# mkangquantum/quits

Measured on AMD Instinct MI355X. Metric: decoded shots/sec + logical-error-rate, [[144,12,12]] BB code, d rounds, p=0.003, higher is better.
Workload: dtype f32

## Files before the change

quits_amd/csrc/bp_scatter_edge.h:

```cpp
#pragma once
#include "qd_internal.h"
#include <float.h>

__device__ __forceinline__ float qs_min_abs(float a, float b)
{
    float r;
    asm("v_min_f32 %0, %1, |%2|" : "=v"(r) : "v"(a), "v"(b));
    return r;
}
typedef uint32_t qs_u32x4 __attribute__((ext_vector_type(4)));
__device__ __forceinline__ uint4 qs_as_uint4(qs_u32x4 v) { return make_uint4(v.x, v.y, v.z, v.w); }
typedef __attribute__((address_space(3))) int32_t qs_lds_i32;
#define QS_LDS(off) ((qs_lds_i32 *)(uintptr_t)(uint32_t)(off))
#define QS_BIG 1.0e30f
#define QS_PRIO 1

#define QS_ACC(off) (*QS_LDS(off))
#define QS_SIGN_TOP (neww & 0x80000000u)
#define QS_HP1(A_) hp ^= (uint32_t)(A_);
#define QS_HPA(A_) hpa = (uint32_t)(A_);
#define QS_HPB(A_) hp = __builtin_amdgcn_bitop3_b32(hp, hpa, (uint32_t)(A_), 0x96);
#define QS_MAG_MASK(q_) (__builtin_amdgcn_inverse_ballot_w64(gsel_ & lq[q_]) ? s2 : s1)
#define QS_EDGE_M(off, k_, SGN_, TAILFIX, HP, MAG_)                                                          \
    {                                                                                                        \
        const int A_ = QS_ACC(off);                                                                          \
        const float mag_ = MAG_;                                                                             \
        const float prev_ = __uint_as_float((SGN_) | __float_as_uint(mag_));                                 \
        float d_ = (float)A_ - prev_;                                                                        \
        TAILFIX(d_, k_)                                                                                      \
        const float bm_ = d_ + 1.0f;                                                                         \
        HP(A_)                                                                                               \
        neww = __builtin_amdgcn_alignbit(neww, __float_as_uint(d_), 31);                                     \
                   \
        asm("v_cmp_lt_f32 vcc, |%1|, %2\n\tv_addc_co_u32 %0, vcc, %0, %0, vcc" : "+v"(ltw) : "v"(bm_), "v"(a1) : "vcc"); \
        a2 = __builtin_amdgcn_fmed3f(a1, a2, fabsf(bm_));                                                    \
        a1 = qs_min_abs(a1, bm_);                                                                            \
    }
__device__ __forceinline__ float qs_min_f32(float a, float b)
{
    float r;
    asm("v_min_f32 %0, %1, %2" : "=v"(r) : "v"(a), "v"(b));
    return r;
}
#define QS_KEY_POS0 0x3F800000u
#define QS_KEY_LIMIT 262144.0f
#define QS_EDGE_K(off, k_, SGN_, TAILFIX, HP, MAG_)                                                          \
    {                                                                                                        \
        const int A_ = QS_ACC(off);                                                                          \
        const float mag_ = MAG_;                                                                             \
        const float prev_ = __uint_as_float((SGN_) | __float_as_uint(mag_));                                 \
        float d_ = (float)A_ - prev_;                                                                        \
        TAILFIX(d_, k_)                                                                                      \
        const float bm_ = d_ + 1.0f;                                                                         \
        HP(A_)                                                                                               \
        neww = __builtin_amdgcn_alignbit(neww, __float_as_uint(d_), 31);                                     \
        const float key_ = fabsf(bm_) + __uint_as_float(QS_KEY_POS0 + ((uint32_t)(k_) << 17));               \
        a2 = __builtin_amdgcn_fmed3f(a1, a2, key_);                                                          \
        a1 = qs_min_f32(a1, key_);                                                                           \
    }
#define QS_KEYS_DECODE(trip_)                                                                                \
    const bool keys_ok_ = __builtin_amdgcn_ballot_w64(!(a2 < QS_KEY_LIMIT)) == 0ull;                         \
    {                                                                                                        \
        const float f1_ = __builtin_floorf(a1), f2_ = __builtin_floorf(a2);                                  \
        kst = min((uint32_t)((a1 - f1_) * 64.0f), (uint32_t)max((trip_) - 1, 0));                            \
        a1 = f1_ - 1.0f; a2 = f2_ - 1.0f;                                                                    \
    }
#define QS_CMP_EDGE QS_EDGE_M
#define QS_CMP_PAD { neww <<= 1; ltw <<= 1; }
#define QS_CMP_WORD_BEGIN uint32_t ltw = 0u;
#define QS_CMP_WORD_END(k0_, kend_) if (ltw) kst = (uint32_t)((k0_) + (kend_) - 1 - (int)__builtin_ctz(ltw));
#define QS_CMP_END(trip_)
#define QS_KEY_EDGE QS_EDGE_K
#define QS_KEY_PAD { neww <<= 1; }
#define QS_KEY_WORD_BEGIN
#define QS_KEY_WORD_END(k0_, kend_)
#define QS_KEY_END(trip_) QS_KEYS_DECODE(trip_)
#define QS_NOFIX(x_, k_)
#define QS_TAILFIX(x_, k_) x_ = ((int)(k_) < dc) ? x_ : QS_BIG;

#define QS_ADD(off, v_) (void)__hip_atomic_fetch_add(QS_LDS(off), v_, __ATOMIC_RELAXED, __HIP_MEMORY_SCOPE_WORKGROUP);
#define QS_SCAT(off, k_, bit_, TAILFIX)                                                                      \
    {                                                                                                        \
        const int sm_ = __builtin_amdgcn_sbfe((int)own, bit_, 1);                                            \
        int v_ = (int)__builtin_amdgcn_bitop3_b32((uint32_t)n1, (uint32_t)nx, (uint32_t)sm_, 0x78);           \
        TAILFIX(v_, k_)                                                                                      \
        QS_ADD(off, v_)                                                                                      \
    }
#define QS_TAILZERO(v_, k_) v_ = ((int)(k_) < dc) ? v_ : 0;

template <int NW>
__device__ __forceinline__ void qs_reset_to_priors(const int32_t *prior_g, uint32_t offA, int nslots, int tid)
{
    const int nbytes = nslots * 4;
    const int lane16 = (tid & 63) * 16;
    for (int p = __builtin_amdgcn_readfirstlane(tid >> 6) * 1024; p < nbytes; p += NW * 1024)
        if (p + lane16 < nbytes)
            __builtin_amdgcn_global_load_lds((const __attribute__((address_space(1))) void *)(reinterpret_cast<const char *>(prior_g) + p + lane16),
                                             (__attribute__((address_space(3))) void *)(uintptr_t)(offA + (uint32_t)p), 16, 0, 0);
}
```

quits_amd/csrc/bp_scatter_wide.hip:

```cpp
#include "qd_internal.h"
#include "qd_host.h"
#include "../../include/quits_amd.h"
#include "bp_scatter_edge.h"

#define QSW_GATHER_PRIO(j_) if ((j_) == 0) __builtin_amdgcn_s_setprio(0); else if ((j_) == CPL - 1) __builtin_amdgcn_s_setprio(2); else __builtin_amdgcn_s_setprio(1);

template <int T, int MW, int CPL, int NSW>
__global__ void __launch_bounds__(T, MW) qd_bp_scatter_wide_kernel(BpGraphDev g, ScatGraphDev sg, DecodeArgs a, ScatArgs x)
{
    extern __shared__ __align__(16) unsigned char smem[];
    const uint32_t lds_base = (uint32_t)(uintptr_t)(__attribute__((address_space(3))) unsigned char *)smem;
    if (lds_base != 0u) __builtin_trap();
    uint32_t *outw = reinterpret_cast<uint32_t *>(smem + sg.off_out);
    int *misc = reinterpret_cast<int *>(smem + sg.off_misc);
    constexpr int NW = T / 64;
    static_assert(T % 64 == 0 && NW <= 16, "workgroup shape");

    const int tid = threadIdx.x;
    const int64_t shot = blockIdx.x;
    const uint8_t *det = a.det + shot * a.det_stride + a.det_offset;
    const uint8_t *upd = a.upd ? a.upd + shot * a.upd_stride : nullptr;
    const int m_pad = g.m_pad, n_pad = g.n_pad;

    int any = 0;
    uint32_t synd[CPL];
    int dcs[CPL];
    bool act[CPL];
    if (tid < 64) misc[tid] = 0;
    int cs[CPL];
#pragma unroll
    for (int j = 0; j < CPL; ++j) {
        const int sw = __builtin_amdgcn_readfirstlane(sg.wave_map[j * NW + (tid >> 6)]);
        const int c = sw * 64 + (tid & 63);
        cs[j] = c;
        act[j] = sw >= 0 && c < g.m;
        synd[j] = 0u; dcs[j] = 0;
        if (act[j]) {
            const uint32_t o = g.chk_orig[c];
            synd[j] = det[o] & 1u;
            if (upd && (int)o < a.upd_rows) synd[j] ^= upd[o] & 1u;
            any |= (int)synd[j];
            dcs[j] = sg.chk_deg[c];
        }
    }
    int dws[CPL];
#pragma unroll
    for (int j = 0; j < CPL; ++j) {
        const int wslot = __builtin_amdgcn_readfirstlane(cs[j] >> 6);
        dws[j] = wslot >= 0 ? (int)sg.deg_w[wslot] : 0;
    }
    qs_reset_to_priors<NW>(x.prior_g, (uint32_t)sg.offA, sg.nslots, tid);
    for (int w = tid; w < g.out_words; w += T) outw[w] = 0u;
    __syncthreads();
    any = qd_block_or(any, misc, NW, 0);
    if (!any) {
        for (int w = tid; w < g.out_words; w += T) a.err_bits[shot * g.out_words + w] = 0u;
        if (tid == 0) a.status[shot] = QD_STATUS_CONVERGED | QD_STATUS_ZERO | a.status_or;
        return;
    }
    float S1[CPL], S2[CPL], A1[CPL], A2[CPL], mx2 = 0.f;
    uint32_t KOLD[CPL], KST[CPL], O[CPL][NSW], Q[CPL][NSW];
    [[maybe_unused]] uint32_t cmpf = 0u;
#pragma unroll
    for (int j = 0; j < CPL; ++j) {
        S1[j] = 0.f; S2[j] = 0.f; A1[j] = FLT_MAX; A2[j] = FLT_MAX; KOLD[j] = 0xFFFFFFFFu; KST[j] = 0u;
#pragma unroll
        for (int w = 0; w < NSW; ++w) { O[j][w] = 0u; Q[j][w] = 0u; }
    }
    const uint32_t cur = (uint32_t)sg.offA;
    const __amdgpu_buffer_rsrc_t adj_rsrc = __builtin_amdgcn_make_buffer_rsrc((void *)sg.adjA, 0, (g.max_rdeg_pad / 4 + 2) * m_pad * 16, 0x00020000);
    const int adj_row = m_pad * 16;
#define QS_ADJ(row_) qs_as_uint4(__builtin_amdgcn_raw_buffer_load_b128(adj_rsrc, adj_voff, (row_) * adj_row, 0))
#define QS_ADJ_FIRST qs_as_uint4(__builtin_amdgcn_raw_buffer_load_b128(adj_rsrc, cs[0] * 16, 0, 0))
    uint4 pf = QS_ADJ_FIRST;
    const bool fast = x.first_pass != nullptr && a.max_iter >= 1;
    bool have = false;
    if (fast) {
#pragma unroll
        for (int j = 0; j < CPL; ++j)
            if (act[j]) {
                const uint4 *rp = reinterpret_cast<const uint4 *>(x.first_pass) + 2 * cs[j];
                const uint4 r0 = rp[0], r1 = rp[1];
                const uint32_t negw[3] = {r0.w, r1.x, r1.y};
                const uint32_t flip = 0u - ((synd[j] ^ r1.z) & 1u);
                A1[j] = __uint_as_float(r0.x); A2[j] = __uint_as_float(r0.y); KST[j] = r0.z;
#pragma unroll
                for (int w = 0; w < NSW; ++w) Q[j][w] = negw[w] ^ flip;
                mx2 = fmaxf(mx2, A2[j]);
            }
        have = true;
    }
#define QSW_VOTE(us_, anyun_)                                                                          \
        {                                                                                              \
            const unsigned long long bal = __ballot(us_);                                              \
            if ((tid & 63) == 0) misc[32 + (tid >> 6)] = (bal != 0ull);                                \
        }                                                                                              \
        __syncthreads();                                                                               \
        anyun_ = 0;                                                                                    \
        {                                                                                              \
            const int4 *f4 = reinterpret_cast<const int4 *>(misc + 32);                                \
            for (int w = 0; w < (NW + 3) / 4; ++w) {                                                   \
                const int4 v = f4[w];                                                                  \
                anyun_ |= v.x | v.y | v.z | v.w;                                                       \
            }                                                                                          \
        }
    int t = 0, converged = 0;
    for (;;) {
      if (!have) {
        bool us = false;
        if (fast && t == a.max_iter) break;
#pragma unroll
        for (int j = 0; j < CPL; ++j) {
            float a1 = FLT_MAX, a2 = FLT_MAX;
            uint32_t kst = 0u;
            QSW_GATHER_PRIO(j)
#define QSW_WALKED                                                                                     \
                {                                                                                      \
                    const uint32_t flip = 0u - ((synd[j] ^ (uint32_t)__popc(par)) & 1u);               \
                    _Pragma("unroll")                                                                  \
                    for (int w = 0; w < NSW; ++w) Q[j][w] = neg[w] ^ flip;                             \
                    mx2 = fmaxf(mx2, a2);                                                              \
                    us = us || (((synd[j] ^ (hp >> 31)) & 1u) != 0u);                                  \
                }
            bool cmpw = true;
            if constexpr (NSW == 2) cmpw = __builtin_amdgcn_ballot_w64((cmpf >> j) & 1u) != 0ull;
#ifdef QSW_STATS
            if ((tid & 63) == 0 && __ballot(act[j])) atomicAdd(&a.dbg[14], 1ull);
#endif
            if (act[j]) {
                if constexpr (NSW == 2) {
                    if (!cmpw) {
#define QS_WALK(p_) QS_KEY_##p_
#include "bp_scatter_wide_walk.inc"
#undef QS_WALK
                        if (keys_ok_) QSW_WALKED
                        else { cmpw = true; cmpf |= 1u << j; a1 = FLT_MAX; a2 = FLT_MAX; kst = 0u; }
                    }
                }
                if (cmpw) {
#ifdef QSW_STATS
                    if ((tid & 63) == 0) atomicAdd(&a.dbg[15], 1ull);
#endif
#define QS_WALK(p_) QS_CMP_##p_
#include "bp_scatter_wide_walk.inc"
#undef QS_WALK
                    QSW_WALKED
                }
            }
#undef QSW_WALKED
            A1[j] = a1; A2[j] = a2; KST[j] = kst;
        }
        __builtin_amdgcn_s_setprio(0);
        pf = QS_ADJ_FIRST;
        int anyun;
        QSW_VOTE(us, anyun)
        if (t >= 1 && !anyun) { converged = 1; break; }
        if (t == a.max_iter) break;
        qs_reset_to_priors<NW>(x.prior_g, cur, sg.nslots, tid);
        __syncthreads();
      }
        have = false;
        __builtin_amdgcn_s_setprio(QS_PRIO);
#pragma unroll
        for (int j = 0; j < CPL; ++j) {
#ifdef QSW_STATS
            {
                bool same = A1[j] == S1[j] && A2[j] == S2[j] && (KST[j] == KOLD[j] || A1[j] == A2[j]);
#pragma unroll
                for (int w = 0; w < NSW; ++w) same = same && Q[j][w] == O[j][w];
                const unsigned long long ba = __ballot(act[j]), bs = __ballot(act[j] && same);
                if ((tid & 63) == 0 && ba) {
                    const int bk = min(t / 10, 4);
                    atomicAdd(&a.dbg[0], 1ull); atomicAdd(&a.dbg[2 + bk], 1ull);
                    if (bs == ba) { atomicAdd(&a.dbg[1], 1ull); atomicAdd(&a.dbg[7 + bk], 1ull); }
                    atomicAdd(&a.dbg[12], (unsigned long long)__popcll(bs)); atomicAdd(&a.dbg[13], (unsigned long long)__popcll(ba));
                }
            }
#endif
            if (act[j]) {
                int dwj = dws[j];
                asm volatile("" : "+s"(dwj));
                const int trip = dwj & 0xFF, wmax = (dwj >> 8) & 0xFF, wmin = (dwj >> 16) & 0xFF, wmin4 = wmin & ~3;
                const int adj_voff = cs[j] * 16;
                const int dc = dcs[j];
                const int n1 = (int)A1[j], nx = n1 ^ -n1;
                const uint32_t kst = KST[j];
                const uint32_t fixn_off = __builtin_amdgcn_raw_buffer_load_b32(adj_rsrc, (int)((kst >> 2) * (uint32_t)adj_row + (kst & 3u) * 4u) + adj_voff, 0, 0);
                const int ng = trip >> 2;
#define QS_GROUP_POS(gi_) const int b0_ = kendw - 1 - 4 * ((gi_) - 8 * w);
#define QS_GROUP_PLAIN(e4, gi_)                                                                                                      \
                {                                                                                                                    \
                    QS_GROUP_POS(gi_)                                                                                                \
                    QS_SCAT(e4.x, 0, b0_, QS_NOFIX) QS_SCAT(e4.y, 0, b0_ - 1, QS_NOFIX) QS_SCAT(e4.z, 0, b0_ - 2, QS_NOFIX) QS_SCAT(e4.w, 0, b0_ - 3, QS_NOFIX) \
                }
#define QS_SCAT_TAIL(off, q_)                                                                                                        \
                    if (k + (q_) < wmin) QS_SCAT(off, 0, b0_ - (q_), QS_NOFIX)                                                       \
                    else if (k + (q_) < wmax) QS_SCAT(off, k + (q_), b0_ - (q_), QS_TAILZERO)
#define QS_GROUP_TAIL(e4, gi_)                                                                                                       \
                {                                                                                                                    \
                    const int k = (gi_) * 4;                                                                                         \
                    QS_GROUP_POS(gi_)                                                                                                \
                    QS_SCAT_TAIL(e4.x, 0) QS_SCAT_TAIL(e4.y, 1) QS_SCAT_TAIL(e4.z, 2) QS_SCAT_TAIL(e4.w, 3)                          \
                }
#pragma unroll
                for (int w = 0; w < NSW; ++w) {
                    if (32 * w < trip) {
                        const int kendw = min(trip - 32 * w, 32);
                        const uint32_t own = Q[j][w];
                        const int g1 = min(ng, 8 * w + 8);
                        const int gp = min(g1, max(wmin4 >> 2, 8 * w));
                        uint4 ea = (j == 0 && w == 0) ? pf : QS_ADJ(8 * w), eb;
                        int gi = 8 * w;
#pragma unroll 1
                        for (; gi + 2 <= gp; gi += 2) {
                            eb = QS_ADJ(gi + 1);
                            QS_GROUP_PLAIN(ea, gi)
                            ea = QS_ADJ(gi + 2);
                            QS_GROUP_PLAIN(eb, gi + 1)
                        }
#pragma unroll 1
                        for (; gi < gp; ++gi) {
                            const uint4 e4 = ea;
                            ea = QS_ADJ(gi + 1);
                            QS_GROUP_PLAIN(e4, gi)
                        }
#pragma unroll 1
                        for (; gi + 1 < g1; ++gi) {
                            const uint4 e4 = ea;
                            ea = QS_ADJ(gi + 1);
                            QS_GROUP_TAIL(e4, gi)
                        }
                        if (gi < g1) QS_GROUP_TAIL(ea, gi)
                    }
                }
#undef QS_GROUP_PLAIN
#undef QS_GROUP_TAIL
#undef QS_SCAT_TAIL
#undef QS_GROUP_POS
                {
                    const int kw = (int)(kst >> 5), kendw = min(trip - 32 * kw, 32);
                    uint32_t wd = Q[j][0];
#pragma unroll
                    for (int w = 1; w < NSW; ++w) wd = (kw == w) ? Q[j][w] : wd;
                    const uint32_t sg_ = (wd >> (kendw - 1 - (int)(kst & 31u))) & 1u;
                    const int dlt = (int)A2[j] - n1;
                    const int vn = sg_ ? -dlt : dlt;
                    (void)__hip_atomic_fetch_add(QS_LDS(fixn_off), vn, __ATOMIC_RELAXED, __HIP_MEMORY_SCOPE_WORKGROUP);
                }
            }
            S1[j] = A1[j]; S2[j] = A2[j]; KOLD[j] = KST[j];
#pragma unroll
            for (int w = 0; w < NSW; ++w) O[j][w] = Q[j][w];
        }
        __builtin_amdgcn_s_setprio(0);
        pf = QS_ADJ_FIRST;
        __syncthreads();
        ++t;
    }
    if (fast && !converged) {
        bool us = false;
#pragma unroll
        for (int j = 0; j < CPL; ++j) {
            QSW_GATHER_PRIO(j)
            if (act[j]) {
                int dwj = dws[j];
                asm volatile("" : "+s"(dwj));
                const int ng = (dwj & 0xFF) >> 2;
                const int adj_voff = cs[j] * 16;
                uint32_t hp = 0u, hpa = 0u;
#define QS_HP_GROUP(e4) { QS_HPA(QS_ACC(e4.x)) QS_HPB(QS_ACC(e4.y)) QS_HPA(QS_ACC(e4.z)) QS_HPB(QS_ACC(e4.w)) }
                uint4 nx = (j == 0) ? pf : QS_ADJ(0);
                int gi = 0;
#pragma unroll 1
                for (; gi + 2 <= ng; gi += 2) {
                    const uint4 eb = QS_ADJ(gi + 1);
                    QS_HP_GROUP(nx)
                    nx = QS_ADJ(gi + 2);
                    QS_HP_GROUP(eb)
                }
                if (gi < ng) QS_HP_GROUP(nx)
#undef QS_HP_GROUP
                us = us || (((synd[j] ^ (hp >> 31)) & 1u) != 0u);
            }
        }
        __builtin_amdgcn_s_setprio(0);
        int anyun;
        QSW_VOTE(us, anyun)
        if (!anyun) converged = 1;
    }
#undef QSW_VOTE
#undef QS_ADJ
#undef QS_ADJ_FIRST
#undef QSW_GATHER_PRIO

    {
        const int tripped = qd_block_or(!(mx2 < x.m2_limit) ? 1 : 0, misc, NW, 0);
        if (tripped) {
            if (tid == 0) {
                const int at = atomicAdd(x.recheck_count, 1);
                if (at < x.recheck_cap) x.recheck_list[at] = (int32_t)shot;
            }
            return;
        }
    }
    for (int b = tid; b < sg.nslots; b += T)
        if (*QS_LDS(cur + 4u * (uint32_t)b) < 0) {
            const uint32_t jf = sg.slot_fault[b];
            if (jf != 0xFFFFFFFFu) atomicOr(&outw[jf >> 5], 1u << (jf & 31u));
        }
    if (!converged && a.want_llr && tid == 0) misc[48] = atomicAdd(a.fail_count, 1);
    __syncthreads();
    for (int w = tid; w < g.out_words; w += T) a.err_bits[shot * g.out_words + w] = outw[w];
    if (!converged && a.want_llr) {
        const int slot = misc[48];
        float *dst = a.llr_ws + (int64_t)slot * n_pad;
        for (int k1 = tid; k1 < g.n; k1 += T) dst[k1] = (float)(*QS_LDS(cur + 4u * sg.k1_slot[k1]) + 1) * x.grid_inv;
        if (tid == 0) a.fail_list[slot] = (int32_t)shot;
    }
    if (tid == 0) a.status[shot] = t | (converged * QD_STATUS_CONVERGED) | a.status_or;
}

#undef QS_ACC
#define QS_ACC(off) (prior_g[((uint32_t)(off) - (uint32_t)sg.offA) >> 2])
#define QS_ADJ(row_) qs_as_uint4(__builtin_amdgcn_raw_buffer_load_b128(adj_rsrc, adj_voff, (row_) * adj_row, 0))
template <int NSW>
__global__ void __launch_bounds__(64) qd_bp_first_pass_kernel(BpGraphDev g, ScatGraphDev sg, const int32_t *prior_g, uint32_t *rec)
{
    static_assert(NSW == 3, "the record has room for three sign words");
    const int c = (int)blockIdx.x * 64 + (int)threadIdx.x;
    const bool actv = c < g.m;
    constexpr int j = 0;
    const int cs[1] = {c}, dws[1] = {__builtin_amdgcn_readfirstlane((int)sg.deg_w[blockIdx.x])}, dcs[1] = {actv ? (int)sg.chk_deg[c] : 0};
    const float S1[1] = {0.f}, S2[1] = {0.f};
    const uint32_t KOLD[1] = {0xFFFFFFFFu}, O[1][NSW] = {{0u, 0u, 0u}};
    const __amdgpu_buffer_rsrc_t adj_rsrc = __builtin_amdgcn_make_buffer_rsrc((void *)sg.adjA, 0, (g.max_rdeg_pad / 4 + 2) * g.m_pad * 16, 0x00020000);
    const int adj_row = g.m_pad * 16;
    const uint4 pf = qs_as_uint4(__builtin_amdgcn_raw_buffer_load_b128(adj_rsrc, c * 16, 0, 0));
    float a1 = FLT_MAX, a2 = FLT_MAX;
    uint32_t kst = 0u;
    uint4 r0 = make_uint4(__float_as_uint(FLT_MAX), __float_as_uint(FLT_MAX), 0u, 0u);
    uint4 r1 = make_uint4(0u, 0u, 0u, (uint32_t)sg.offA + (uint32_t)(sg.nslots - 32 + (int)(threadIdx.x & 31)) * 4u);
    if (actv) {
#define QS_WALK(p_) QS_CMP_##p_
#include "bp_scatter_wide_walk.inc"
#undef QS_WALK
        (void)hp;
        r0 = make_uint4(__float_as_uint(a1), __float_as_uint(a2), kst, neg[0]);
        r1 = make_uint4(neg[1], neg[2], (uint32_t)__popc(par) & 1u,
                        __builtin_amdgcn_raw_buffer_load_b32(adj_rsrc, (int)((kst >> 2) * (uint32_t)adj_row + (kst & 3u) * 4u) + c * 16, 0, 0));
    }
    uint4 *out = reinterpret_cast<uint4 *>(rec) + 2 * c;
    out[0] = r0; out[1] = r1;
}
#undef QS_ADJ
#undef QS_ACC

hipError_t qd_launch_bp_first_pass(const BpGraphDev &g, const ScatGraphDev &sg, const int32_t *prior_g, uint32_t *rec, hipStream_t s)
{
    if (g.max_rdeg_pad > 96 || g.m_pad % 64) return hipErrorInvalidValue;
    hipLaunchKernelGGL(qd_bp_first_pass_kernel<3>, dim3((unsigned)(g.m_pad / 64)), dim3(64), 0, s, g, sg, prior_g, rec);
    return hipGetLastError();
}

template <int T, int MW, int CPL, int NSW>
static hipError_t launch_scatter_wide_t(const BpGraphDev &g, const ScatGraphDev &sg, const DecodeArgs &a, const ScatArgs &x, int64_t B, hipStream_t s)
{
    auto k = qd_bp_scatter_wide_kernel<T, MW, CPL, NSW>;
    hipError_t e = hipFuncSetAttribute((const void *)k, hipFuncAttributeMaxDynamicSharedMemorySize, sg.lds_bytes);
    if (e != hipSuccess) return e;
    hipLaunchKernelGGL(k, dim3((unsigned)B), dim3(T), sg.lds_bytes, s, g, sg, a, x);
    return hipGetLastError();
}

hipError_t qd_launch_bp_scatter_wide(const BpGraphDev &g, const ScatGraphDev &sg, const DecodeArgs &a, const ScatArgs &x, int64_t B, hipStream_t s)
{
    const bool two_words = g.max_rdeg_pad <= 64;
    switch (sg.wide_threads * 8 + sg.wide_cpl) {
    case 512 * 8 + 2:
        return two_words ? launch_scatter_wide_t<512, 8, 2, 2>(g, sg, a, x, B, s) : hipErrorInvalidValue;
    case 256 * 8 + 2:
        return two_words ? launch_scatter_wide_t<256, 8, 2, 2>(g, sg, a, x, B, s) : hipErrorInvalidValue;
    case 128 * 8 + 2:
        return two_words ? launch_scatter_wide_t<128, 8, 2, 2>(g, sg, a, x, B, s) : hipErrorInvalidValue;
    case 256 * 8 + 1:
        return two_words ? launch_scatter_wide_t<256, 8, 1, 2>(g, sg, a, x, B, s) : hipErrorInvalidValue;
    case 512 * 8 + 1:
        return two_words ? launch_scatter_wide_t<512, 8, 1, 2>(g, sg, a, x, B, s) : hipErrorInvalidValue;
    case 1024 * 8 + 1:
        return two_words ? launch_scatter_wide_t<1024, 8, 1, 2>(g, sg, a, x, B, s) : hipErrorInvalidValue;
    case 704 * 8 + 2:
        return launch_scatter_wide_t<704, 6, 2, 3>(g, sg, a, x, B, s);
    case 1024 * 8 + 2: return launch_scatter_wide_t<1024, 4, 2, 3>(g, sg, a, x, B, s);
    case 512 * 8 + 3: return launch_scatter_wide_t<512, 4, 3, 3>(g, sg, a, x, B, s);
    default: return hipErrorInvalidValue;
    }
}
```

Baseline: 1.824 million.

## Merge per-check state arrays, prefetch fix address, and streamline convergence vote

Drops the separate A1/A2/KST/Q state arrays and writes gather results directly into S1/S2/KOLD/O, which removes the end-of-iteration copy and reduces register pressure. The fix-node LDS address load is issued early, after the gather phase and before the barrier, instead of inside the scatter phase. The syndrome is stored in the sign bit so the unsatisfied-check vote becomes a single bitop3 and a sign-bit ballot, and the cross-wave vote read is reduced to one int2/int4 load. The signed fix-up uses an sbfe mask instead of a branch. The risk is subtle correctness changes in the reworked bit-position and sign logic.

Measured after the change: 1.855 million, median of 6. 1.7% higher.

```diff
diff --git a/quits_amd/csrc/bp_scatter_edge.h b/quits_amd/csrc/bp_scatter_edge.h
--- a/quits_amd/csrc/bp_scatter_edge.h
+++ b/quits_amd/csrc/bp_scatter_edge.h
@@ -40,6 +40,12 @@
 {
     float r;
     asm("v_min_f32 %0, %1, %2" : "=v"(r) : "v"(a), "v"(b));
+    return r;
+}
+__device__ __forceinline__ float qs_max_f32(float a, float b)
+{
+    float r;
+    asm("v_max_f32 %0, %1, %2" : "=v"(r) : "v"(a), "v"(b));
     return r;
 }
 #define QS_KEY_POS0 0x3F800000u
diff --git a/quits_amd/csrc/bp_scatter_wide.hip b/quits_amd/csrc/bp_scatter_wide.hip
--- a/quits_amd/csrc/bp_scatter_wide.hip
+++ b/quits_amd/csrc/bp_scatter_wide.hip
@@ -39,6 +39,7 @@
             const uint32_t o = g.chk_orig[c];
             synd[j] = det[o] & 1u;
             if (upd && (int)o < a.upd_rows) synd[j] ^= upd[o] & 1u;
+            synd[j] <<= 31;
             any |= (int)synd[j];
             dcs[j] = sg.chk_deg[c];
         }
@@ -58,20 +59,31 @@
         if (tid == 0) a.status[shot] = QD_STATUS_CONVERGED | QD_STATUS_ZERO | a.status_or;
         return;
     }
-    float S1[CPL], S2[CPL], A1[CPL], A2[CPL], mx2 = 0.f;
-    uint32_t KOLD[CPL], KST[CPL], O[CPL][NSW], Q[CPL][NSW];
+    float S1[CPL], S2[CPL], mx2 = 0.f;
+    uint32_t KOLD[CPL], O[CPL][NSW];
+    uint32_t FX[CPL];
+#ifdef QSW_STATS
+    float P1[CPL], P2[CPL];
+    uint32_t PK[CPL], PO[CPL][NSW];
+#endif
     [[maybe_unused]] uint32_t cmpf = 0u;
 #pragma unroll
     for (int j = 0; j < CPL; ++j) {
-        S1[j] = 0.f; S2[j] = 0.f; A1[j] = FLT_MAX; A2[j] = FLT_MAX; KOLD[j] = 0xFFFFFFFFu; KST[j] = 0u;
-#pragma unroll
-        for (int w = 0; w < NSW; ++w) { O[j][w] = 0u; Q[j][w] = 0u; }
+        S1[j] = 0.f; S2[j] = 0.f; KOLD[j] = 0xFFFFFFFFu; FX[j] = 0u;
+#pragma unroll
+        for (int w = 0; w < NSW; ++w) O[j][w] = 0u;
+#ifdef QSW_STATS
+        P1[j] = 0.f; P2[j] = 0.f; PK[j] = 0xFFFFFFFFu;
+#pragma unroll
+        for (int w = 0; w < NSW; ++w) PO[j][w] = 0u;
+#endif
     }
     const uint32_t cur = (uint32_t)sg.offA;
     const __amdgpu_buffer_rsrc_t adj_rsrc = __builtin_amdgcn_make_buffer_rsrc((void *)sg.adjA, 0, (g.max_rdeg_pad / 4 + 2) * m_pad * 16, 0x00020000);
     const int adj_row = m_pad * 16;
 #define QS_ADJ(row_) qs_as_uint4(__builtin_amdgcn_raw_buffer_load_b128(adj_rsrc, adj_voff, (row_) * adj_row, 0))
 #define QS_ADJ_FIRST qs_as_uint4(__builtin_amdgcn_raw_buffer_load_b128(adj_rsrc, cs[0] * 16, 0, 0))
+#define QS_FIX_ADDR(j_) __builtin_amdgcn_raw_buffer_load_b32(adj_rsrc, (int)(__umul24(KOLD[j_] >> 2, (uint32_t)adj_row) + (KOLD[j_] & 3u) * 4u) + cs[j_] * 16, 0, 0)
     uint4 pf = QS_ADJ_FIRST;
     const bool fast = x.first_pass != nullptr && a.max_iter >= 1;
     bool have = false;
@@ -82,32 +94,32 @@
                 const uint4 *rp = reinterpret_cast<const uint4 *>(x.first_pass) + 2 * cs[j];
                 const uint4 r0 = rp[0], r1 = rp[1];
                 const uint32_t negw[3] = {r0.w, r1.x, r1.y};
-                const uint32_t flip = 0u - ((synd[j] ^ r1.z) & 1u);
-                A1[j] = __uint_as_float(r0.x); A2[j] = __uint_as_float(r0.y); KST[j] = r0.z;
-#pragma unroll
-                for (int w = 0; w < NSW; ++w) Q[j][w] = negw[w] ^ flip;
-                mx2 = fmaxf(mx2, A2[j]);
+                const uint32_t flip = 0u - (((synd[j] >> 31) ^ r1.z) & 1u);
+                S1[j] = __uint_as_float(r0.x); S2[j] = __uint_as_float(r0.y); KOLD[j] = r0.z; FX[j] = r1.w;
+#pragma unroll
+                for (int w = 0; w < NSW; ++w) O[j][w] = negw[w] ^ flip;
+                mx2 = qs_max_f32(mx2, S2[j]);
             }
         have = true;
     }
-#define QSW_VOTE(us_, anyun_)                                                                          \
+#define QSW_VOTE_ROUND(uw_, synd_, hp_) uw_ = __builtin_amdgcn_bitop3_b32(uw_, synd_, hp_, 0xF6);
+#define QSW_VOTE(uw_, anyun_)                                                                          \
         {                                                                                              \
-            const unsigned long long bal = __ballot(us_);                                              \
-            if ((tid & 63) == 0) misc[32 + (tid >> 6)] = (bal != 0ull);                                \
+            const unsigned long long bal = __ballot((int)(uw_) < 0);                                   \
+            if ((tid & 63) == 0) reinterpret_cast<unsigned char *>(misc + 32)[tid >> 6] = (unsigned char)(bal != 0ull); \
         }                                                                                              \
         __syncthreads();                                                                               \
-        anyun_ = 0;                                                                                    \
-        {                                                                                              \
-            const int4 *f4 = reinterpret_cast<const int4 *>(misc + 32);                                \
-            for (int w = 0; w < (NW + 3) / 4; ++w) {                                                   \
-                const int4 v = f4[w];                                                                  \
-                anyun_ |= v.x | v.y | v.z | v.w;                                                       \
-            }                                                                                          \
+        if constexpr (NW <= 8) {                                                                       \
+            const int2 v = *reinterpret_cast<const int2 *>(misc + 32);                                 \
+            anyun_ = v.x | v.y;                                                                        \
+        } else {                                                                                       \
+            const int4 v = *reinterpret_cast<const int4 *>(misc + 32);                                 \
+            anyun_ = (v.x | v.y) | (v.z | v.w);                                                        \
         }
     int t = 0, converged = 0;
     for (;;) {
       if (!have) {
-        bool us = false;
+        uint32_t us = 0u;
         if (fast && t == a.max_iter) break;
 #pragma unroll
         for (int j = 0; j < CPL; ++j) {
@@ -116,16 +128,19 @@
             QSW_GATHER_PRIO(j)
 #define QSW_WALKED                                                                                     \
                 {                                                                                      \
-                    const uint32_t flip = 0u - ((synd[j] ^ (uint32_t)__popc(par)) & 1u);               \
+                    const uint32_t flip = 0u - ((uint32_t)__popc(par ^ synd[j]) & 1u);                 \
                     _Pragma("unroll")                                                                  \
-                    for (int w = 0; w < NSW; ++w) Q[j][w] = neg[w] ^ flip;                             \
-                    mx2 = fmaxf(mx2, a2);                                                              \
-                    us = us || (((synd[j] ^ (hp >> 31)) & 1u) != 0u);                                  \
+                    for (int w = 0; w < NSW; ++w) O[j][w] = neg[w] ^ flip;                             \
+                    mx2 = qs_max_f32(mx2, a2);                                                         \
+                    QSW_VOTE_ROUND(us, synd[j], hp)                                                    \
                 }
             bool cmpw = true;
             if constexpr (NSW == 2) cmpw = __builtin_amdgcn_ballot_w64((cmpf >> j) & 1u) != 0ull;
 #ifdef QSW_STATS
             if ((tid & 63) == 0 && __ballot(act[j])) atomicAdd(&a.dbg[14], 1ull);
+            P1[j] = S1[j]; P2[j] = S2[j]; PK[j] = KOLD[j];
+#pragma unroll
+            for (int w = 0; w < NSW; ++w) PO[j][w] = O[j][w];
 #endif
             if (act[j]) {
                 if constexpr (NSW == 2) {
@@ -148,10 +163,13 @@
                 }
             }
 #undef QSW_WALKED
-            A1[j] = a1; A2[j] = a2; KST[j] = kst;
+            S1[j] = a1; S2[j] = a2; KOLD[j] = kst;
         }
         __builtin_amdgcn_s_setprio(0);
         pf = QS_ADJ_FIRST;
+#pragma unroll
+        for (int j = 0; j < CPL; ++j)
+            if (act[j]) FX[j] = QS_FIX_ADDR(j);
         int anyun;
         QSW_VOTE(us, anyun)
         if (t >= 1 && !anyun) { converged = 1; break; }
@@ -165,9 +183,9 @@
         for (int j = 0; j < CPL; ++j) {
 #ifdef QSW_STATS
             {
-                bool same = A1[j] == S1[j] && A2[j] == S2[j] && (KST[j] == KOLD[j] || A1[j] == A2[j]);
-#pragma unroll
-                for (int w = 0; w < NSW; ++w) same = same && Q[j][w] == O[j][w];
+                bool same = S1[j] == P1[j] && S2[j] == P2[j] && (KOLD[j] == PK[j] || S1[j] == S2[j]);
+#pragma unroll
+                for (int w = 0; w < NSW; ++w) same = same && O[j][w] == PO[j][w];
                 const unsigned long long ba = __ballot(act[j]), bs = __ballot(act[j] && same);
                 if ((tid & 63) == 0 && ba) {
                     const int bk = min(t / 10, 4);
@@ -183,9 +201,9 @@
                 const int trip = dwj & 0xFF, wmax = (dwj >> 8) & 0xFF, wmin = (dwj >> 16) & 0xFF, wmin4 = wmin & ~3;
                 const int adj_voff = cs[j] * 16;
                 const int dc = dcs[j];
-                const int n1 = (int)A1[j], nx = n1 ^ -n1;
-                const uint32_t kst = KST[j];
-                const uint32_t fixn_off = __builtin_amdgcn_raw_buffer_load_b32(adj_rsrc, (int)((kst >> 2) * (uint32_t)adj_row + (kst & 3u) * 4u) + adj_voff, 0, 0);
+                const int n1 = (int)S1[j], nx = n1 ^ -n1;
+                const uint32_t kst = KOLD[j];
+                const uint32_t fixn_off = FX[j];
                 const int ng = trip >> 2;
 #define QS_GROUP_POS(gi_) const int b0_ = kendw - 1 - 4 * ((gi_) - 8 * w);
 #define QS_GROUP_PLAIN(e4, gi_)                                                                                                      \
@@ -206,7 +224,7 @@
                 for (int w = 0; w < NSW; ++w) {
                     if (32 * w < trip) {
                         const int kendw = min(trip - 32 * w, 32);
-                        const uint32_t own = Q[j][w];
+                        const uint32_t own = O[j][w];
                         const int g1 = min(ng, 8 * w + 8);
                         const int gp = min(g1, max(wmin4 >> 2, 8 * w));
                         uint4 ea = (j == 0 && w == 0) ? pf : QS_ADJ(8 * w), eb;
@@ -238,19 +256,20 @@
 #undef QS_SCAT_TAIL
 #undef QS_GROUP_POS
                 {
-                    const int kw = (int)(kst >> 5), kendw = min(trip - 32 * kw, 32);
-                    uint32_t wd = Q[j][0];
-#pragma unroll
-                    for (int w = 1; w < NSW; ++w) wd = (kw == w) ? Q[j][w] : wd;
-                    const uint32_t sg_ = (wd >> (kendw - 1 - (int)(kst & 31u))) & 1u;
-                    const int dlt = (int)A2[j] - n1;
-                    const int vn = sg_ ? -dlt : dlt;
+                    uint32_t wd = O[j][0];
+                    int bpos = min(trip, 32) - 1 - (int)kst;
+#pragma unroll
+                    for (int w = 1; w < NSW; ++w) {
+                        const bool inw = kst >= 32u * (uint32_t)w;
+                        wd = inw ? O[j][w] : wd;
+                        bpos = inw ? min(trip - 32 * w, 32) - 1 + 32 * w - (int)kst : bpos;
+                    }
+                    const int m_ = __builtin_amdgcn_sbfe((int)wd, bpos, 1);
+                    const int dlt = (int)S2[j] - n1;
+                    const int vn = (dlt ^ m_) - m_;
                     (void)__hip_atomic_fetch_add(QS_LDS(fixn_off), vn, __ATOMIC_RELAXED, __HIP_MEMORY_SCOPE_WORKGROUP);
                 }
             }
-            S1[j] = A1[j]; S2[j] = A2[j]; KOLD[j] = KST[j];
-#pragma unroll
-            for (int w = 0; w < NSW; ++w) O[j][w] = Q[j][w];
         }
         __builtin_amdgcn_s_setprio(0);
         pf = QS_ADJ_FIRST;
@@ -258,7 +277,7 @@
         ++t;
     }
     if (fast && !converged) {
-        bool us = false;
+        uint32_t us = 0u;
 #pragma unroll
         for (int j = 0; j < CPL; ++j) {
             QSW_GATHER_PRIO(j)
@@ -280,7 +299,7 @@
                 }
                 if (gi < ng) QS_HP_GROUP(nx)
 #undef QS_HP_GROUP
-                us = us || (((synd[j] ^ (hp >> 31)) & 1u) != 0u);
+                QSW_VOTE_ROUND(us, synd[j], hp)
             }
         }
         __builtin_amdgcn_s_setprio(0);
@@ -289,8 +308,10 @@
         if (!anyun) converged = 1;
     }
 #undef QSW_VOTE
+#undef QSW_VOTE_ROUND
 #undef QS_ADJ
 #undef QS_ADJ_FIRST
+#undef QS_FIX_ADDR
 #undef QSW_GATHER_PRIO
 
     {
```
